# gpuopenanalytics/libgdf

Hardware: AMD Instinct MI355X
Metric: hash-join probe rows/s (higher is better)
Workload: dtype int64

## Files before the change

### libgdf_amd/csrc/join.hip

```cpp
#include "internal.h"
#include "launch.h"
#include "gdf/gdf_amd_ext.h"

#include <cmath>
#include <cstdio>

#include <algorithm>
#include <cstdlib>
#include <deque>
#include <memory>
#include <type_traits>
#include <vector>

namespace gdf_amd {

enum KeyMode : int { KM_RAW_INT = 0, KM_RAW_FLOAT, KM_PACKED, KM_HASHED };

struct KeyPlan {
  int mode;
  int verify;
  int narrow;
  uint64_t kmin;
  uint64_t kspan;
  uint64_t klimit;
// ... 1215 lines not shown
      tiles = (next - first + tile - 1) / tile;
    }
    uint32_t total;
    const uint32_t before = bk_block_scan<uint32_t>(tiles, lds_wave, &total);
    if (c < ncoarse) { coarse_off[c] = first; tile_prefix[c] = run + before; }
    run += total;
    block_sync();
  }
  if (threadIdx.x == 0) { coarse_off[ncoarse] = total_rows; tile_prefix[ncoarse] = run; }
  for (uint32_t f = threadIdx.x; f < nfine; f += JK_BK_THREADS) cursor[f] = begin[f];
}

struct Unit {
  uint32_t build_begin, build_count;
  uint32_t probe_begin, probe_count;
};

__global__ __launch_bounds__(256) void jk_make_units(uint32_t nfine, uint32_t cap2, const uint32_t *__restrict__ cursor,
                                                     const uint32_t *__restrict__ level1_flag,
                                                     const uint32_t *__restrict__ build_begin, const uint32_t *__restrict__ build_cnt,
                                                     int keep_probe, Unit *__restrict__ units, uint64_t *__restrict__ off,
                                                     unsigned long long *__restrict__ state, const uint32_t *__restrict__ fstart = nullptr,
                                                     const uint32_t *__restrict__ fcap = nullptr) {
  const uint32_t f = blockIdx.x * 256 + threadIdx.x;
  const uint32_t fc = f < nfine ? f : nfine - 1;
  const uint32_t cur = cursor[fc], bn = build_cnt[fc], bb = build_begin[fc];
  const uint32_t first = fstart ? fstart[fc] : fc * cap2;
  if (fcap) cap2 = fcap[fc];
  const uint32_t grown = f < nfine ? cur - first : 0u;
  const uint32_t all = grown < cap2 ? grown : cap2;
  const uint32_t pn = (all != 0 && (bn != 0 || keep_probe)) ? all : 0u;
  const uint32_t nun = (pn + JK_PROBE_CHUNK - 1) / JK_PROBE_CHUNK;
  const uint32_t incl_u = wave_scan_incl(nun);
  const unsigned long long incl_t = wave_scan_incl((unsigned long long)pn);
  const unsigned long long sum_all = wave_reduce_add((unsigned long long)all);
  unsigned long long base_u = 0, base_t = 0;
  if (lane_id() == WAVE - 1) {
    if (incl_u) { base_u = atomicAdd(&state[0], (unsigned long long)incl_u); base_t = atomicAdd(&state[1], incl_t); }
    if (sum_all) atomicAdd(&state[2], sum_all);
  }
  base_u = __shfl(base_u, WAVE - 1, WAVE);
  base_t = __shfl(base_t, WAVE - 1, WAVE);
  unsigned long long u = base_u + incl_u - nun, o = base_t + incl_t - pn;
  for (uint32_t at = 0; at < pn; at += JK_PROBE_CHUNK) {
    const uint32_t cnt = pn - at < JK_PROBE_CHUNK ? pn - at : JK_PROBE_CHUNK;
    units[u] = Unit{bb, bn, first + at, cnt};
    off[u] = o;
    ++u;
    o += cnt;
  }
  if (f == 0) state[3] = (unsigned long long)((cursor[nfine] ? 1u : 0u) | ((level1_flag && *level1_flag) ? 2u : 0u));
}

struct ProbeArgs {
  Tuples build, probe;
  const Unit *units;
  uint32_t nslots;
  uint32_t cap;
  int keep_unmatched_probe;
  int verify;
  uint8_t *build_matched;
  uint64_t *counts;
  int32_t *out_probe; int32_t *out_build;
  int unused;
  uint64_t kbias;
  int optimistic;
  unsigned long long *opt_state;
  uint32_t *unit_todo;
  uint32_t sample_n;
  const unsigned long long *nunits_dev;
  uint32_t *unit_pairs;
  int pay_mode;
  const void *pay_src[2];
  void *pay_out[2];
  int key_width;
  const void *key_src;
  void *key_out;
  int bpay_mode;
  const void *bpay_src[2];
  void *bpay_out[2];
  int p6_fb;
  uint32_t p6_world;
  uint64_t p6_kbias;
};
__device__ __forceinline__ void pay_gather(const ProbeArgs &a, unsigned long long pos, int32_t prow) {
  if (a.pay_mode == 1 || a.pay_mode == 4) {
    ((uint64_t *)a.pay_out[0])[pos] = ((const uint64_t *)a.pay_src[0])[prow];
    if (a.pay_mode == 4) ((uint64_t *)a.pay_out[1])[pos] = ((const uint64_t *)a.pay_src[1])[prow];
  } else if (a.pay_mode) {
    ((uint32_t *)a.pay_out[0])[pos] = ((const uint32_t *)a.pay_src[0])[prow];
    if (a.pay_mode == 3) ((uint32_t *)a.pay_out[1])[pos] = ((const uint32_t *)a.pay_src[1])[prow];
  }
  if (a.key_width == 8) ((uint64_t *)a.key_out)[pos] = ((const uint64_t *)a.key_src)[prow];
  else if (a.key_width == 4) ((uint32_t *)a.key_out)[pos] = ((const uint32_t *)a.key_src)[prow];
}
__device__ __forceinline__ void bpay_gather(const ProbeArgs &a, unsigned long long pos, int32_t brow) {
  if (a.bpay_mode == 1 || a.bpay_mode == 4) {
    ((uint64_t *)a.bpay_out[0])[pos] = ((const uint64_t *)a.bpay_src[0])[brow];
    if (a.bpay_mode == 4) ((uint64_t *)a.bpay_out[1])[pos] = ((const uint64_t *)a.bpay_src[1])[brow];
  } else if (a.bpay_mode) {
    ((uint32_t *)a.bpay_out[0])[pos] = ((const uint32_t *)a.bpay_src[0])[brow];
    if (a.bpay_mode == 3) ((uint32_t *)a.bpay_out[1])[pos] = ((const uint32_t *)a.bpay_src[1])[brow];
  }
}

struct ProbeLds {
  uint64_t *bw;
  uint32_t *T;
  int32_t *bi;
  unsigned long long *wave_cnt;
  unsigned long long *unit_cursor;
  unsigned int *cuckoo_failed;
  uint32_t *next;
};

template <bool NARROW>
__device__ __forceinline__ ProbeLds carve_probe_lds(unsigned char *raw, uint32_t cap, uint32_t H) {
  ProbeLds l;
  l.bw = (uint64_t *)raw;
  l.T = (uint32_t *)(raw + (size_t)cap * 8);
  unsigned char *after = raw + (size_t)cap * 8 + (size_t)H * 8;
  l.bi = (int32_t *)after;
  if (!NARROW) after += (size_t)cap * 4;
  l.wave_cnt = (unsigned long long *)after;
  l.unit_cursor = l.wave_cnt + JK_PROBE_THREADS / WAVE;
  l.cuckoo_failed = (unsigned int *)(l.unit_cursor + 1);
  l.next = (uint32_t *)(l.unit_cursor + 2);
  return l;
}
static size_t probe_lds_bytes(bool narrow, uint32_t cap, uint32_t H, bool chained = true) {
  return (size_t)cap * (narrow ? 8 : 12) + (size_t)H * 8 + sizeof(unsigned long long) * (JK_PROBE_THREADS / WAVE + 2) +
         (chained ? (size_t)cap * 4 : 0);
}

template <bool NARROW>
__device__ __forceinline__ int32_t build_row(const ProbeLds &l, uint32_t p) {
  return NARROW ? (int32_t)(uint32_t)l.bw[p] : l.bi[p];
}

template <bool WRITE, bool NARROW, bool P6 = false>
__global__ __launch_bounds__(JK_PROBE_THREADS) void jk_probe(ProbeArgs a, KeyTable probe_t, KeyTable build_t) {
  extern __shared__ __attribute__((aligned(16))) unsigned char lds_raw[];
  const uint32_t H = a.nslots, cap = a.cap;
  const ProbeLds l = carve_probe_lds<NARROW>(lds_raw, cap, H);
  uint32_t uid = a.unit_todo ? a.unit_todo[blockIdx.x] : blockIdx.x;
  if (a.sample_n) {
    const unsigned long long nunits = *a.nunits_dev;
    if (nunits == 0) return;
    uid = (uint32_t)(((unsigned long long)blockIdx.x * nunits) / a.sample_n);
  }
  const Unit u = a.units[uid];

  for (uint32_t i = threadIdx.x; i < u.build_count; i += JK_PROBE_THREADS) {
    uint64_t w = a.build.w[u.build_begin + i];
    if constexpr (P6 && NARROW) w = ((uint64_t)p6_remainder((uint32_t)(w >> 32), a.p6_kbias, a.p6_fb, a.p6_world) << 32) | (uint32_t)w;
    else if constexpr (P6) w = p10_key(w + a.p6_kbias, a.p6_fb);
    l.bw[i] = w;
    if (!NARROW) l.bi[i] = a.build.idx[u.build_begin + i];
  }
  for (uint32_t i = threadIdx.x; i < 2 * H; i += JK_PROBE_THREADS) l.T[i] = JK_NOPOS;
  __shared__ uint32_t dup_seen;
  if (threadIdx.x == 0) { *l.unit_cursor = WRITE ? a.counts[uid] : 0ull; *l.cuckoo_failed = 0; dup_seen = 0; }
  block_sync();

  for (uint32_t p0 = threadIdx.x; p0 < u.build_count; p0 += JK_PROBE_THREADS) {
    uint32_t cur = p0, table = 0;
// ... 140 lines not shown
          }
        }
      }
    }
#pragma unroll
    for (int b = 0; b < NB; ++b) {
      const bool active = act[b];
      uint32_t c = cnt[b];
      const bool pad = active && c == 0 && a.keep_unmatched_probe;
      if (pad) c = 1;
      if (!WRITE) {
        my_count += c;
      } else {
        unsigned long long pos;
        if (__all(c <= 1)) {
          const unsigned long long mm = __ballot(c == 1);
          unsigned long long wbase = 0;
          if (lane_id() == 0 && mm) wbase = atomicAdd(l.unit_cursor, (unsigned long long)__popcll(mm));
          pos = __shfl(wbase, 0, WAVE) + mask_rank(mm);
        } else {
          const uint32_t incl = wave_scan_incl(c);
          const uint32_t wave_total = __shfl(incl, WAVE - 1, WAVE);
          unsigned long long wbase = 0;
          if (lane_id() == 0) wbase = atomicAdd(l.unit_cursor, (unsigned long long)wave_total);
          pos = __shfl(wbase, 0, WAVE) + incl - c;
        }
        if (pos + c > unit_end) {
          if (c) a.opt_state[1] = 1;
        } else if (pad) {
          a.out_probe[pos] = prow[b];
          a.out_build[pos] = JK_EMPTY;
          pay_gather(a, pos, prow[b]);
        } else if (c >= 1 && (cuckoo || c == 1)) {
          a.out_probe[pos] = prow[b];
          a.out_build[pos] = build_row<NARROW>(l, hit_a[b]);
          pay_gather(a, pos, prow[b]);
          bpay_gather(a, pos, build_row<NARROW>(l, hit_a[b]));
          if (c == 2) {
            a.out_probe[pos + 1] = prow[b];
            a.out_build[pos + 1] = build_row<NARROW>(l, hit_b[b]);
            pay_gather(a, pos + 1, prow[b]);
            bpay_gather(a, pos + 1, build_row<NARROW>(l, hit_b[b]));
          }
        } else if (c > 1) {
          for (uint32_t p = hit_b[b]; p != JK_NOPOS; p = l.next[p]) {
            if (!a.verify || rows_equal(probe_t, prow[b], build_t, build_row<NARROW>(l, p))) {
              a.out_probe[pos] = prow[b];
              a.out_build[pos] = build_row<NARROW>(l, p);
              pay_gather(a, pos, prow[b]);
              bpay_gather(a, pos, build_row<NARROW>(l, p));
              ++pos;
            }
          }
        }
      }
    }
  }
  if (WRITE && a.optimistic) {
    block_sync();
    if (threadIdx.x == 0) {
      atomicAdd(&a.opt_state[0], *l.unit_cursor - unit_base);
      if (a.unit_pairs) a.unit_pairs[uid] = (uint32_t)(*l.unit_cursor - unit_base);
    }
  }
  if (!WRITE) {
    my_count = wave_reduce_add(my_count);
    if (lane_id() == 0) l.wave_cnt[threadIdx.x / WAVE] = my_count;
    block_sync();
    if (threadIdx.x == 0) {
      unsigned long long t = 0;
      for (int w = 0; w < JK_PROBE_THREADS / WAVE; ++w) t += l.wave_cnt[w];
      if (a.sample_n) { atomicAdd(&a.opt_state[0], t); atomicAdd(&a.opt_state[1], (unsigned long long)u.probe_count); }
      else a.counts[uid] = t;
    }
  }
}

template <bool POW2, bool KEEP, bool NARROW, int PMODE = 0, bool P6 = false>
__global__ __launch_bounds__(JK_PROBE_THREADS) void jk_probe_fast(ProbeArgs a) {
  extern __shared__ __attribute__((aligned(16))) unsigned char lds_raw[];
  const uint32_t H = a.nslots, cap = a.cap;
  const ProbeLds l = carve_probe_lds<NARROW>(lds_raw, cap, H);
  unsigned int *lcur = (unsigned int *)l.unit_cursor;
  const Unit u = a.units[blockIdx.x];
  for (uint32_t i = threadIdx.x; i < u.build_count; i += JK_PROBE_THREADS) {
    uint64_t w = a.build.w[u.build_begin + i];
    if constexpr (P6 && NARROW) w = ((uint64_t)p6_remainder((uint32_t)(w >> 32), a.p6_kbias, a.p6_fb, a.p6_world) << 32) | (uint32_t)w;
    else if constexpr (P6) w = p10_key(w + a.p6_kbias, a.p6_fb);
    l.bw[i] = w;
    if (!NARROW) l.bi[i] = a.build.idx[u.build_begin + i];
  }
  for (uint32_t i = threadIdx.x; i < 2 * H; i += JK_PROBE_THREADS) l.T[i] = JK_NOPOS;
  if (threadIdx.x == 0) { *lcur = 0; *l.cuckoo_failed = 0; }
  block_sync();
  const uint32_t kb_lo = (uint32_t)a.kbias, kb_hi = (uint32_t)(a.kbias >> 32);
  using Key = typename std::conditional<NARROW, uint32_t, uint64_t>::type;
  auto fold_of = [&](Key key) -> uint32_t {
    if constexpr (P6 && !NARROW) {
      uint32_t x = (uint32_t)(key >> 32);
      x ^= x << 13;
      x ^= x >> 7;
      return x ^ (uint32_t)key;
    } else if constexpr (P6) {
      uint32_t x = (uint32_t)key;
      x ^= x << 13;
      x ^= x >> 7;
      return x;
    } else if constexpr (NARROW) {
      const uint32_t lo = key + kb_lo;
      const uint32_t hi = kb_hi + (lo < key ? 1u : 0u);
      return lo ^ (hi * 0x9e3779b1u);
    } else {
      return key_fold(key + a.kbias);
    }
  };
  auto fold2_of = [&](Key key, uint32_t f1) -> uint32_t {
    if constexpr (NARROW) return f1;
    else if constexpr (P6) {
      uint32_t x = (uint32_t)(key >> 32);
      x ^= x << 13;
      x ^= x >> 7;
      return __builtin_rotateleft32(x, 16) + (uint32_t)key + ((uint32_t)key << 3);
    } else return key_fold2(key + a.kbias);
  };
  auto staged_key = [&](uint32_t p) -> Key {
    if constexpr (NARROW) return (uint32_t)(l.bw[p] >> 32);
    else return l.bw[p];
  };
  const int hshift = POW2 ? 32 - (__ffs((int)H) - 1) : 0;
  uint32_t seed = 0;
  for (int attempt = 0; attempt < 4; ++attempt) {
    for (uint32_t p0 = threadIdx.x; p0 < u.build_count; p0 += JK_PROBE_THREADS) {
      uint32_t cur = p0, table = 0;
      int moves = 0;
      for (; moves < JK_CUCKOO_MAX_MOVES; ++moves) {
        const Key ck = staged_key(cur);
        const uint32_t f = fold_of(ck) ^ seed, f2 = fold2_of(ck, fold_of(ck)) ^ seed;
        const uint32_t slot = table ? H + (POW2 ? (f2 * 0xc2b2ae35u) >> hshift : __umulhi(f2 * 0xc2b2ae35u, H))
                                    : (POW2 ? (f * 0x9e3779b1u) >> hshift : __umulhi(f * 0x9e3779b1u, H));
        const uint32_t old = atomicExch(&l.T[slot], cur);
        if (old == JK_NOPOS) break;
        cur = old;
        table ^= 1;
      }
      if (moves == JK_CUCKOO_MAX_MOVES) *l.cuckoo_failed = 1;
    }
    block_sync();
    if (!*l.cuckoo_failed || attempt == 3) break;
    block_sync();
    for (uint32_t i = threadIdx.x; i < 2 * H; i += JK_PROBE_THREADS) l.T[i] = JK_NOPOS;
    if (threadIdx.x == 0) *l.cuckoo_failed = 0;
    seed += 0x9e3779b9u;
    block_sync();
  }
  if (*l.cuckoo_failed) {
    if (threadIdx.x == 0) a.unit_todo[atomicAdd(&a.opt_state[2], 1ull)] = blockIdx.x;
    return;
  }
  const unsigned long long unit_base = a.counts[blockIdx.x];
  const uint32_t unit_cap = a.optimistic ? u.probe_count : 0xffffffffu;
  int32_t *__restrict__ op = a.out_probe + unit_base;
  int32_t *__restrict__ ob = a.out_build + unit_base;
  constexpr int NB = JK_PROBE_BATCH * 2;
  const uint32_t lead = u.probe_begin & 1u;
  const uint64_t *__restrict__ src = a.probe.w + (u.probe_begin - lead);
  const int32_t *__restrict__ src_row = NARROW ? nullptr : a.probe.idx + (u.probe_begin - lead);
  const uint64_t *__restrict__ src_pay = PMODE ? a.probe.pay + (size_t)(u.probe_begin - lead) * (PMODE == 4 ? 2 : 1) : nullptr;
  uint64_t *__restrict__ po8 = (PMODE == 1 || PMODE == 4) ? (uint64_t *)a.pay_out[0] + unit_base : nullptr;
  uint64_t *__restrict__ po8b = PMODE == 4 ? (uint64_t *)a.pay_out[1] + unit_base : nullptr;
  uint32_t *__restrict__ po4a = (PMODE == 2 || PMODE == 3) ? (uint32_t *)a.pay_out[0] + unit_base : nullptr;
  uint32_t *__restrict__ po4b = PMODE == 3 ? (uint32_t *)a.pay_out[1] + unit_base : nullptr;
  uint64_t *__restrict__ ko8 = (PMODE && a.key_width == 8) ? (uint64_t *)a.key_out + unit_base : nullptr;
  uint32_t *__restrict__ ko4 = (PMODE && a.key_width == 4) ? (uint32_t *)a.key_out + unit_base : nullptr;
  const uint32_t vtotal = lead + u.probe_count;
  const uint32_t last_pair = (vtotal - 1) & ~1u;
  for (uint32_t base = 0; base < vtotal; base += JK_PROBE_THREADS * NB) {
    Key key[NB];
    uint32_t prow[NB];
    uint64_t pay[PMODE ? NB : 1], pay2[PMODE == 4 ? NB : 1];
    bool act[NB];
#pragma unroll
    for (int b = 0; b < JK_PROBE_BATCH; ++b) {
      const uint32_t v = base + (b * JK_PROBE_THREADS + threadIdx.x) * 2;
      const uint32_t vc = v < last_pair ? v : last_pair;
      ulonglong2 ww{};
      if constexpr (P6) {
        uint32_t r0, row0, r1, row1;
        p6_load_pair(a.probe.w, (u.probe_begin - lead) + vc, r0, row0, r1, row1);
        if constexpr (NARROW) {
          key[2 * b] = r0; key[2 * b + 1] = r1;
        } else {
          const HiPair hh = *reinterpret_cast<const HiPair *>(a.probe.idx + (u.probe_begin - lead) + vc);
          key[2 * b] = ((uint64_t)r0 << 32) | hh.a; key[2 * b + 1] = ((uint64_t)r1 << 32) | hh.b;
        }
        prow[2 * b] = row0; prow[2 * b + 1] = row1;
      } else {
        ww = *reinterpret_cast<const ulonglong2 *>(src + vc);
      }
      if constexpr (PMODE == 4) {
        const ulonglong2 p0 = *reinterpret_cast<const ulonglong2 *>(src_pay + 2 * (size_t)vc);
        const ulonglong2 p1 = *reinterpret_cast<const ulonglong2 *>(src_pay + 2 * (size_t)vc + 2);
        pay[2 * b] = p0.x; pay2[2 * b] = p0.y; pay[2 * b + 1] = p1.x; pay2[2 * b + 1] = p1.y;
      } else if constexpr (PMODE != 0) {
        const ulonglong2 pp = *reinterpret_cast<const ulonglong2 *>(src_pay + vc);
        pay[2 * b] = pp.x; pay[2 * b + 1] = pp.y;
      }
      if constexpr (P6) {
      } else if constexpr (NARROW) {
        key[2 * b] = (uint32_t)(ww.x >> 32); prow[2 * b] = (uint32_t)ww.x;
        key[2 * b + 1] = (uint32_t)(ww.y >> 32); prow[2 * b + 1] = (uint32_t)ww.y;
      } else {
        const uint2 rr = *reinterpret_cast<const uint2 *>(src_row + vc);
        key[2 * b] = ww.x; prow[2 * b] = rr.x;
        key[2 * b + 1] = ww.y; prow[2 * b + 1] = rr.y;
      }
      act[2 * b] = v >= lead && v < vtotal;
      act[2 * b + 1] = v + 1 < vtotal;
    }
    uint32_t pa[NB], pb[NB];
#pragma unroll
    for (int b = 0; b < NB; ++b) {
      const uint32_t f = fold_of(key[b]) ^ seed, f2 = fold2_of(key[b], fold_of(key[b])) ^ seed;
      pa[b] = l.T[POW2 ? (f * 0x9e3779b1u) >> hshift : __umulhi(f * 0x9e3779b1u, H)];
      pb[b] = l.T[H + (POW2 ? (f2 * 0xc2b2ae35u) >> hshift : __umulhi(f2 * 0xc2b2ae35u, H))];
    }
    uint64_t wa[NB], wb[NB];
#pragma unroll
    for (int b = 0; b < NB; ++b) {
      wa[b] = l.bw[pa[b] == JK_NOPOS ? 0 : pa[b]];
      wb[b] = l.bw[pb[b] == JK_NOPOS ? 0 : pb[b]];
    }
    uint32_t hamask = 0, hbmask = 0, padmask = 0;
#pragma unroll
    for (int b = 0; b < NB; ++b) {
      const bool ha = act[b] && pa[b] != JK_NOPOS && (NARROW ? (uint32_t)(wa[b] >> 32) == (uint32_t)key[b] : wa[b] == (uint64_t)key[b]);
      const bool hb = act[b] && pb[b] != JK_NOPOS && (NARROW ? (uint32_t)(wb[b] >> 32) == (uint32_t)key[b] : wb[b] == (uint64_t)key[b]);
      hamask |= (uint32_t)ha << b;
      hbmask |= (uint32_t)hb << b;
      padmask |= (uint32_t)(KEEP && act[b] && !ha && !hb) << b;
    }
    int32_t hitrow[NARROW ? 1 : NB];
    if constexpr (!NARROW) {
#pragma unroll
      for (int b = 0; b < NB; ++b) {
        const bool ha = (hamask >> b) & 1u, hb = (hbmask >> b) & 1u;
        hitrow[b] = l.bi[ha ? pa[b] : (hb ? pb[b] : 0u)];
      }
    }
    auto emit = [&](int b, uint32_t pos, uint32_t c) {
      const bool ha = (hamask >> b) & 1u, pad = (padmask >> b) & 1u;
      if (pos + c > unit_cap) a.opt_state[1] = 1;
      else {
        int32_t first;
        if constexpr (NARROW) first = ha ? (int32_t)(uint32_t)wa[b] : (int32_t)(uint32_t)wb[b];
        else first = hitrow[b];
        op[pos] = (int32_t)prow[b];
        ob[pos] = pad ? JK_EMPTY : first;
        if (c == 2) {
          op[pos + 1] = (int32_t)prow[b];
          if constexpr (NARROW) ob[pos + 1] = (int32_t)(uint32_t)wb[b];
          else ob[pos + 1] = l.bi[pb[b]];
        }
        if constexpr (PMODE == 1 || PMODE == 4) { po8[pos] = pay[b]; if (c == 2) po8[pos + 1] = pay[b]; }
        if constexpr (PMODE == 4) { po8b[pos] = pay2[b]; if (c == 2) po8b[pos + 1] = pay2[b]; }
        if constexpr (PMODE == 2 || PMODE == 3) { po4a[pos] = (uint32_t)pay[b]; if (c == 2) po4a[pos + 1] = (uint32_t)pay[b]; }
        if constexpr (PMODE == 3) { po4b[pos] = (uint32_t)(pay[b] >> 32); if (c == 2) po4b[pos + 1] = (uint32_t)(pay[b] >> 32); }
        if constexpr (PMODE != 0 && NARROW) {
          if (ko8) { ko8[pos] = (uint64_t)key[b] + a.kbias; if (c == 2) ko8[pos + 1] = (uint64_t)key[b] + a.kbias; }
          if (ko4) { ko4[pos] = (uint32_t)key[b]; if (c == 2) ko4[pos + 1] = (uint32_t)key[b]; }
        }
      }
    };
    if (__all((hamask & hbmask) == 0)) {
      const uint32_t onemask = hamask | hbmask | padmask;
      unsigned long long mm[NB];
      uint32_t off[NB], tot = 0;
#pragma unroll
      for (int b = 0; b < NB; ++b) {
        mm[b] = __ballot((onemask >> b) & 1u);
        off[b] = tot;
        tot += (uint32_t)__popcll(mm[b]);
      }
      uint32_t wbase = 0;
      if (lane_id() == 0 && tot) wbase = atomicAdd(lcur, tot);
      wbase = (uint32_t)__builtin_amdgcn_readfirstlane((int)wbase);
#pragma unroll
      for (int b = 0; b < NB; ++b)
        if ((onemask >> b) & 1u) emit(b, wbase + off[b] + (uint32_t)mask_rank(mm[b]), 1u);
    } else {
#pragma unroll
      for (int b = 0; b < NB; ++b) {
        const uint32_t c = ((hamask >> b) & 1u) + ((hbmask >> b) & 1u) + ((padmask >> b) & 1u);
        uint32_t pos;
        if (__all(c <= 1)) {
          const unsigned long long mm = __ballot(c == 1);
          uint32_t wbase = 0;
          if (lane_id() == 0 && mm) wbase = atomicAdd(lcur, (unsigned int)__popcll(mm));
          pos = __shfl(wbase, 0, WAVE) + mask_rank(mm);
        } else {
          const uint32_t incl = wave_scan_incl(c);
          const uint32_t wave_total = __shfl(incl, WAVE - 1, WAVE);
          uint32_t wbase = 0;
          if (lane_id() == 0) wbase = atomicAdd(lcur, wave_total);
          pos = __shfl(wbase, 0, WAVE) + incl - c;
        }
        if (c) emit(b, pos, c);
      }
    }
  }
  if (a.optimistic) {
    block_sync();
    if (threadIdx.x == 0) {
      atomicAdd(&a.opt_state[0], (unsigned long long)*lcur);
      if (a.unit_pairs) a.unit_pairs[blockIdx.x] = *lcur;
    }
  }
}

template <bool POW2, bool KEEP, bool NARROW, bool P6 = false>
__global__ __launch_bounds__(JK_PROBE_THREADS) void jk_count_fast(ProbeArgs a) {
  extern __shared__ __attribute__((aligned(16))) unsigned char lds_raw[];
  const uint32_t H = a.nslots, cap = a.cap;
  const ProbeLds l = carve_probe_lds<NARROW>(lds_raw, cap, H);
  const Unit u = a.units[blockIdx.x];
  for (uint32_t i = threadIdx.x; i < u.build_count; i += JK_PROBE_THREADS) {
    uint64_t w = a.build.w[u.build_begin + i];
    if constexpr (P6 && NARROW) w = ((uint64_t)p6_remainder((uint32_t)(w >> 32), a.p6_kbias, a.p6_fb, a.p6_world) << 32) | (uint32_t)w;
    else if constexpr (P6) w = p10_key(w + a.p6_kbias, a.p6_fb);
    l.bw[i] = w;
    if (!NARROW) l.bi[i] = a.build.idx[u.build_begin + i];
  }
  for (uint32_t i = threadIdx.x; i < 2 * H; i += JK_PROBE_THREADS) l.T[i] = JK_NOPOS;
  if (threadIdx.x == 0) *l.cuckoo_failed = 0;
  block_sync();
  const uint32_t kb_lo = (uint32_t)a.kbias, kb_hi = (uint32_t)(a.kbias >> 32);
  using Key = typename std::conditional<NARROW, uint32_t, uint64_t>::type;
  auto fold_of = [&](Key key) -> uint32_t {
    if constexpr (P6 && !NARROW) {
      uint32_t x = (uint32_t)(key >> 32);
      x ^= x << 13;
      x ^= x >> 7;
      return x ^ (uint32_t)key;
    } else if constexpr (P6) {
      uint32_t x = (uint32_t)key;
      x ^= x << 13;
      x ^= x >> 7;
      return x;
    } else if constexpr (NARROW) {
      const uint32_t lo = key + kb_lo;
      const uint32_t hi = kb_hi + (lo < key ? 1u : 0u);
      return lo ^ (hi * 0x9e3779b1u);
    } else {
      return key_fold(key + a.kbias);
    }
  };
  auto fold2_of = [&](Key key, uint32_t f1) -> uint32_t {
    if constexpr (NARROW) return f1;
    else if constexpr (P6) {
      uint32_t x = (uint32_t)(key >> 32);
      x ^= x << 13;
      x ^= x >> 7;
      return __builtin_rotateleft32(x, 16) + (uint32_t)key + ((uint32_t)key << 3);
    } else return key_fold2(key + a.kbias);
  };
  auto staged_key = [&](uint32_t p) -> Key {
    if constexpr (NARROW) return (uint32_t)(l.bw[p] >> 32);
    else return l.bw[p];
  };
  const int hshift = POW2 ? 32 - (__ffs((int)H) - 1) : 0;
  uint32_t seed = 0;
  for (int attempt = 0; attempt < 4; ++attempt) {
    for (uint32_t p0 = threadIdx.x; p0 < u.build_count; p0 += JK_PROBE_THREADS) {
      uint32_t cur = p0, table = 0;
      int moves = 0;
      for (; moves < JK_CUCKOO_MAX_MOVES; ++moves) {
        const Key ck = staged_key(cur);
        const uint32_t f = fold_of(ck) ^ seed, f2 = fold2_of(ck, fold_of(ck)) ^ seed;
        const uint32_t slot = table ? H + (POW2 ? (f2 * 0xc2b2ae35u) >> hshift : __umulhi(f2 * 0xc2b2ae35u, H))
                                    : (POW2 ? (f * 0x9e3779b1u) >> hshift : __umulhi(f * 0x9e3779b1u, H));
        const uint32_t old = atomicExch(&l.T[slot], cur);
        if (old == JK_NOPOS) break;
        cur = old;
        table ^= 1;
      }
      if (moves == JK_CUCKOO_MAX_MOVES) *l.cuckoo_failed = 1;
    }
    block_sync();
    if (!*l.cuckoo_failed || attempt == 3) break;
    block_sync();
// ... 1225 lines not shown
    sb->pay[0].reset();
    if (flag) return GDF_SUCCESS;
    if (app) {
      app->rows += n;
      *ok = true;
      return GDF_SUCCESS;
    }
    sb->fine_begin.resize(nfine);
    sb->fine_cnt.resize(nfine);
    for (uint32_t f = 0; f < nfine; ++f) { sb->fine_begin[f] = f * cap2; sb->fine_cnt[f] = cur[f] - f * cap2; }
    sb->final_buf = 1;
  }
  uint64_t total = 0;
  for (uint32_t c : sb->fine_cnt) total += c;
  sb->joinable = (uint32_t)total;
  sb->speculative = true;
  *ok = true;
  return GDF_SUCCESS;
}

static gdf_error spec_append_finish(const PartGeom &g, SpecAppend *app, SideBufs *sb) {
  const uint32_t nfine = 1u << g.fb;
  std::vector<uint32_t> cur(nfine);
  HIP_TRY(read_back(cur.data(), app->cursor.p, sizeof(uint32_t) * nfine));
  sb->fine_off.clear();
  sb->fine_begin.resize(nfine);
  sb->fine_cnt.resize(nfine);
  uint64_t total = 0;
  for (uint32_t f = 0; f < nfine; ++f) {
    sb->fine_begin[f] = f * app->cap2;
    sb->fine_cnt[f] = cur[f] - f * app->cap2;
    total += sb->fine_cnt[f];
  }
  sb->final_buf = 1;
  sb->joinable = (uint32_t)total;
  sb->speculative = true;
  return GDF_SUCCESS;
}

static gdf_error run_probe(bool narrow, bool write, const char *name, size_t nunits, size_t lds, const ProbeArgs &a,
                           const KeyTable &probe_t, const KeyTable &build_t) {
  if (!nunits) return GDF_SUCCESS;
  GDF_TRY(with_bools([&](auto W, auto N, auto P6) {
    return launch_lds(name, jk_probe<W(), N(), P6()>, dim3((unsigned)nunits), dim3(JK_PROBE_THREADS), lds, a, probe_t, build_t);
  }, write, narrow, a.p6_fb != 0));
  HIP_CHECK_LAST();
  return GDF_SUCCESS;
}

static bool lean_table(uint32_t max_build, ProbeArgs *fa) {
  const bool pow2 = (double)max_build <= 0.42 * 2.0 * (double)fa->nslots;
  if (!pow2) fa->nslots = ((uint32_t)(max_build * 1.25) + 63) & ~63u;
  return pow2;
}

static gdf_error run_write_pass(bool narrow, bool plain, size_t nunits, size_t lds, ProbeArgs a, uint32_t max_build,
                                const KeyTable &probe_t, const KeyTable &build_t) {
  if (!nunits) return GDF_SUCCESS;
  if (!plain)
    return run_probe(narrow, true, "jk_probe_write", nunits, lds, a, probe_t, build_t);
  DevBuf todo;
  RMM_TRY(todo.alloc(sizeof(uint32_t) * nunits));
  a.unit_todo = todo.as<uint32_t>();
  ProbeArgs fa = a;
  const bool pow2 = lean_table(max_build, &fa);
  const size_t flds = probe_lds_bytes(narrow, a.cap, fa.nslots, false);
  const bool keep = a.keep_unmatched_probe != 0;
  auto lean = [&](auto N, auto M, auto P6) {
    return with_bools([&](auto P2, auto KP) {
      return launch_lds("jk_probe_write", jk_probe_fast<P2(), KP(), N(), M(), P6()>, dim3((unsigned)nunits), dim3(JK_PROBE_THREADS), flds, fa);
    }, pow2, keep);
  };
  constexpr std::true_type yes{};
  constexpr std::false_type no{};
  constexpr std::integral_constant<int, 0> none{};
  if (narrow && a.bpay_mode && !keep) {
    const bool bw2 = a.bpay_mode == 4;
    const size_t blds = probe_bp_lds_bytes(a.cap, fa.nslots, bw2);
    GDF_TRY(with_bools([&](auto P2, auto B2) {
      return with_int<0, 1, 2>(pay_words(a.pay_mode), [&](auto PP) {
        return launch_lds("jk_probe_write", jk_probe_bp<P2(), PP(), B2()>, dim3((unsigned)nunits), dim3(JK_BP_THREADS), blds, fa);
      });
    }, pow2, bw2));
  } else if (narrow && a.p6_fb) {
    GDF_TRY(lean(yes, none, yes));
  } else if (narrow && a.pay_mode) {
    GDF_TRY(with_int<1, 2, 3, 4>(a.pay_mode, [&](auto M) { return lean(yes, M, no); }));
  } else if (narrow) {
    GDF_TRY(lean(yes, none, no));
  } else {
    GDF_TRY(with_bools([&](auto P6) { return lean(no, none, P6); }, a.p6_fb != 0));
  }
  HIP_CHECK_LAST();
  unsigned long long left = 0;
  HIP_TRY(read_back(&left, a.opt_state + 2, sizeof(left)));
  if (left) GDF_TRY(run_probe(narrow, true, "jk_probe_write_general", (size_t)left, lds, a, probe_t, build_t));
  HIP_TRY(hipStreamSynchronize(stream0()));
  return GDF_SUCCESS;
}

static gdf_error run_multi_pass(bool write, size_t nunits, size_t lds, const ProbeArgs &a) {
  if (!nunits) return GDF_SUCCESS;
  GDF_TRY(with_bools([&](auto W, auto KP, auto SIX) {
    return launch_lds(write ? "jk_probe_write" : "jk_probe_count", jk_probe_multi<W(), KP(), SIX()>, dim3((unsigned)nunits), dim3(JK_PROBE_THREADS), lds, a);
  }, write, a.keep_unmatched_probe != 0, a.p6_fb != 0));
  HIP_CHECK_LAST();
  return GDF_SUCCESS;
}

static gdf_error run_count_pass(bool narrow, bool plain, size_t nunits, size_t lds, ProbeArgs a, uint32_t max_build,
                                const KeyTable &probe_t, const KeyTable &build_t) {
  if (!nunits) return GDF_SUCCESS;
  if (!plain || a.build_matched)
    return run_probe(narrow, false, "jk_probe_count", nunits, lds, a, probe_t, build_t);
  DevBuf todo;
  RMM_TRY(todo.alloc(sizeof(uint32_t) * nunits));
  a.unit_todo = todo.as<uint32_t>();
  ProbeArgs fa = a;
  const bool pow2 = lean_table(max_build, &fa);
  const size_t flds = probe_lds_bytes(narrow, a.cap, fa.nslots, false);
  GDF_TRY(with_bools([&](auto P2, auto KP, auto N, auto P6) {
    return launch_lds("jk_probe_count", jk_count_fast<P2(), KP(), N(), P6()>, dim3((unsigned)nunits), dim3(JK_PROBE_THREADS), flds, fa);
  }, pow2, a.keep_unmatched_probe != 0, narrow, a.p6_fb != 0));
  HIP_CHECK_LAST();
  unsigned long long left = 0;
  HIP_TRY(read_back(&left, a.opt_state + 2, sizeof(left)));
  if (left) GDF_TRY(run_probe(narrow, false, "jk_probe_count_general", (size_t)left, lds, a, probe_t, build_t));
  HIP_TRY(hipStreamSynchronize(stream0()));
  return GDF_SUCCESS;
}

static gdf_error refine_side(const PartGeom &g, bool narrow, double dup, SideBufs *sb, bool *ok) {
  *ok = false;
  const uint32_t nseg = 1u << g.fb, nsub = 1u << g.b3;
  const uint64_t nfine3 = (uint64_t)nseg << g.b3;
  const int64_t n = sb->joinable;
  if (n == 0) return GDF_SUCCESS;
  const int64_t TILE = (int64_t)JK_SC2_THREADS * (sb->pay[sb->final_buf].p ? JK_PAY_ITEMS : JK_SC_ITEMS);
  const double mean = (double)n / (double)nfine3;
  const uint32_t cap3 = (uint32_t)(((uint64_t)(mean + 8.0 * std::sqrt(mean * (1.0 + dup)) + 64.0) + 7) / 8 * 8);
  const uint64_t size3 = nfine3 * cap3 + TILE;
  if (size3 >= 0x7fffffffULL) return GDF_SUCCESS;
  std::vector<uint32_t> seg(2 * (size_t)nseg), tile_prefix((size_t)nseg + 1), cur((size_t)nfine3);
  tile_prefix[0] = 0;
  for (uint32_t c = 0; c < nseg; ++c) {
    seg[c] = sb->fine_begin[c];
    seg[nseg + c] = sb->fine_begin[c] + sb->fine_cnt[c];
    tile_prefix[c + 1] = tile_prefix[c] + (uint32_t)((sb->fine_cnt[c] + TILE - 1) / TILE);
  }
  for (uint64_t f = 0; f < nfine3; ++f) cur[f] = (uint32_t)(f * cap3);
  const uint32_t ntiles = tile_prefix[nseg];
  DevBuf d_seg, d_tiles, cursor, flag, nw, nidx, npay;
  const bool carries = sb->pay[sb->final_buf].p != nullptr;
  RMM_TRY(d_seg.alloc(sizeof(uint32_t) * 2 * nseg));
  RMM_TRY(d_tiles.alloc(sizeof(uint32_t) * ((size_t)nseg + 1)));
  RMM_TRY(cursor.alloc(sizeof(uint32_t) * nfine3));
  RMM_TRY(flag.alloc(sizeof(uint32_t)));
  RMM_TRY(nw.alloc(sizeof(uint64_t) * size3));
  if (!narrow) RMM_TRY(nidx.alloc(sizeof(int32_t) * size3));
  if (carries) RMM_TRY(npay.alloc(sizeof(uint64_t) * sb->pay_words * size3));
  HIP_TRY(hipMemcpyAsync(d_seg.p, seg.data(), sizeof(uint32_t) * 2 * nseg, hipMemcpyHostToDevice, stream0()));
  HIP_TRY(hipMemcpyAsync(d_tiles.p, tile_prefix.data(), sizeof(uint32_t) * ((size_t)nseg + 1), hipMemcpyHostToDevice, stream0()));
  HIP_TRY(hipMemcpyAsync(cursor.p, cur.data(), sizeof(uint32_t) * nfine3, hipMemcpyHostToDevice, stream0()));
  HIP_TRY(hipMemsetAsync(flag.p, 0, sizeof(uint32_t), stream0()));
  PartGeom g3 = g;
  g3.b1 = g.fb;
// ... 1881 lines not shown
```

Measured before the change: 109.9 billion.

## Add bitmap-rank probe kernel replacing cuckoo table for dense narrow keys

Adds a probe kernel that builds a per-unit LDS bitmap with prefix counts over key remainders, so each probe is a direct bit test plus popcount rank instead of a two-table cuckoo lookup. Units whose remainders collide fall back to the existing cuckoo kernel through a new unit list, and then to the general path. The aim is to remove cuckoo insertion cost and double-slot probing. The trade-offs are a large fixed LDS footprint, which lowers residency, and an extra readback and launch whenever any unit has duplicate remainders.

Measured after the change: 103.1 billion. -6.3%, worse.

```diff
diff --git a/libgdf_amd/csrc/join.hip b/libgdf_amd/csrc/join.hip
--- a/libgdf_amd/csrc/join.hip
+++ b/libgdf_amd/csrc/join.hip
@@ -1321,6 +1321,7 @@
   int p6_fb;
   uint32_t p6_world;
   uint64_t p6_kbias;
+  const uint32_t *unit_list;
 };
 __device__ __forceinline__ void pay_gather(const ProbeArgs &a, unsigned long long pos, int32_t prow) {
   if (a.pay_mode == 1 || a.pay_mode == 4) {
@@ -1627,7 +1628,8 @@
   const uint32_t H = a.nslots, cap = a.cap;
   const ProbeLds l = carve_probe_lds<NARROW>(lds_raw, cap, H);
   unsigned int *lcur = (unsigned int *)l.unit_cursor;
-  const Unit u = a.units[blockIdx.x];
+  const uint32_t uid = a.unit_list ? a.unit_list[blockIdx.x] : blockIdx.x;
+  const Unit u = a.units[uid];
   for (uint32_t i = threadIdx.x; i < u.build_count; i += JK_PROBE_THREADS) {
     uint64_t w = a.build.w[u.build_begin + i];
     if constexpr (P6 && NARROW) w = ((uint64_t)p6_remainder((uint32_t)(w >> 32), a.p6_kbias, a.p6_fb, a.p6_world) << 32) | (uint32_t)w;
@@ -1699,10 +1701,10 @@
     block_sync();
   }
   if (*l.cuckoo_failed) {
-    if (threadIdx.x == 0) a.unit_todo[atomicAdd(&a.opt_state[2], 1ull)] = blockIdx.x;
+    if (threadIdx.x == 0) a.unit_todo[atomicAdd(&a.opt_state[2], 1ull)] = uid;
     return;
   }
-  const unsigned long long unit_base = a.counts[blockIdx.x];
+  const unsigned long long unit_base = a.counts[uid];
   const uint32_t unit_cap = a.optimistic ? u.probe_count : 0xffffffffu;
   int32_t *__restrict__ op = a.out_probe + unit_base;
   int32_t *__restrict__ ob = a.out_build + unit_base;
@@ -1850,6 +1852,189 @@
           pos = __shfl(wbase, 0, WAVE) + incl - c;
         }
         if (c) emit(b, pos, c);
+      }
+    }
+  }
+  if (a.optimistic) {
+    block_sync();
+    if (threadIdx.x == 0) {
+      atomicAdd(&a.opt_state[0], (unsigned long long)*lcur);
+      if (a.unit_pairs) a.unit_pairs[uid] = *lcur;
+    }
+  }
+}
+
+constexpr int JK_RANK_BITS = 32 - JK_MAX_FB;
+constexpr uint32_t JK_RANK_WORDS = 1u << (JK_RANK_BITS - 5);
+constexpr int JK_RANK_STAGE = (JK_MAX_BUILD + JK_PROBE_THREADS - 1) / JK_PROBE_THREADS;
+constexpr bool JK_RANK_PACKED = false;
+constexpr int JK_RANK_BATCH = 4;
+constexpr int JK_RANK_RESIDENT = 2;
+static_assert(JK_RANK_WORDS % JK_PROBE_THREADS == 0 && JK_RANK_WORDS / JK_PROBE_THREADS == 8, "a thread owns 8 consecutive bitmap words");
+static_assert(JK_MAX_BUILD <= 0xffff, "the prefix of a bitmap word is a u16");
+static size_t rank_lds_bytes(uint32_t cap, bool packed) {
+  return (size_t)JK_RANK_WORDS * (packed ? 8 : 6) + (size_t)cap * 4 + sizeof(uint32_t) * (JK_PROBE_THREADS / WAVE + 4);
+}
+static size_t rank_launch_lds(uint32_t cap, bool packed) {
+  return std::max(rank_lds_bytes(cap, packed), (size_t)160 * 1024 / (JK_RANK_RESIDENT + 1) + 64);
+}
+template <bool KEEP, bool PACKED>
+__global__ __launch_bounds__(JK_PROBE_THREADS) void jk_probe_rank(ProbeArgs a) {
+  extern __shared__ __attribute__((aligned(16))) unsigned char lds_raw[];
+  constexpr int WORDS_PER_THREAD = JK_RANK_WORDS / JK_PROBE_THREADS;
+  uint2 *ent = (uint2 *)lds_raw;
+  uint32_t *bits = (uint32_t *)lds_raw;
+  uint16_t *pre = (uint16_t *)(lds_raw + (size_t)JK_RANK_WORDS * 4);
+  int32_t *brow = (int32_t *)(lds_raw + (size_t)JK_RANK_WORDS * (PACKED ? 8 : 6));
+  uint32_t *wave_sum = (uint32_t *)(brow + a.cap);
+  unsigned int *lcur = wave_sum + JK_PROBE_THREADS / WAVE;
+  unsigned int *repeated = lcur + 1;
+  const Unit u = a.units[blockIdx.x];
+  const uint32_t room = a.cap < (uint32_t)(JK_RANK_STAGE * JK_PROBE_THREADS) ? a.cap : (uint32_t)(JK_RANK_STAGE * JK_PROBE_THREADS);
+  const uint32_t bn = u.build_count < room ? u.build_count : room;
+  uint64_t bw[JK_RANK_STAGE];
+  if (bn) {
+#pragma unroll
+    for (int k = 0; k < JK_RANK_STAGE; ++k) {
+      const uint32_t i = k * JK_PROBE_THREADS + threadIdx.x;
+      bw[k] = a.build.w[u.build_begin + (i < bn ? i : bn - 1)];
+    }
+  } else {
+#pragma unroll
+    for (int k = 0; k < JK_RANK_STAGE; ++k) bw[k] = 0;
+  }
+  const uint32_t w0 = threadIdx.x * WORDS_PER_THREAD;
+  if constexpr (PACKED) {
+#pragma unroll
+    for (int j = 0; j < WORDS_PER_THREAD; j += 2) *reinterpret_cast<uint4 *>(&ent[w0 + j]) = uint4{0, 0, 0, 0};
+  } else {
+    *reinterpret_cast<uint4 *>(&bits[w0]) = uint4{0, 0, 0, 0};
+    *reinterpret_cast<uint4 *>(&bits[w0 + 4]) = uint4{0, 0, 0, 0};
+  }
+  if (threadIdx.x == 0) { *lcur = 0; *repeated = 0; }
+  block_sync();
+  uint32_t rem[JK_RANK_STAGE];
+  bool twice = false;
+#pragma unroll
+  for (int k = 0; k < JK_RANK_STAGE; ++k) {
+    rem[k] = p6_remainder((uint32_t)(bw[k] >> 32), a.p6_kbias, a.p6_fb, a.p6_world);
+    if (k * JK_PROBE_THREADS + threadIdx.x < bn) {
+      const uint32_t bit = 1u << (rem[k] & 31u);
+      const uint32_t old = PACKED ? atomicOr(&ent[rem[k] >> 5].x, bit) : atomicOr(&bits[rem[k] >> 5], bit);
+      twice |= (old & bit) != 0;
+    }
+  }
+  if (twice) *repeated = 1;
+  block_sync();
+  if (*repeated) {
+    if (threadIdx.x == 0) a.unit_todo[atomicAdd(&a.opt_state[3], 1ull)] = blockIdx.x;
+    return;
+  }
+  {
+    uint32_t wd[WORDS_PER_THREAD], mine = 0;
+#pragma unroll
+    for (int j = 0; j < WORDS_PER_THREAD; ++j) {
+      wd[j] = PACKED ? ent[w0 + j].x : bits[w0 + j];
+      mine += (uint32_t)__popc(wd[j]);
+    }
+    const uint32_t incl = wave_scan_incl(mine);
+    if (lane_id() == WAVE - 1) wave_sum[threadIdx.x / WAVE] = incl;
+    block_sync();
+    uint32_t run = incl - mine;
+#pragma unroll
+    for (int w = 0; w < JK_PROBE_THREADS / WAVE; ++w)
+      if (w < (int)(threadIdx.x / WAVE)) run += wave_sum[w];
+    if constexpr (PACKED) {
+#pragma unroll
+      for (int j = 0; j < WORDS_PER_THREAD; ++j) {
+        ent[w0 + j].y = run;
+        run += (uint32_t)__popc(wd[j]);
+      }
+    } else {
+      uint32_t packed[WORDS_PER_THREAD / 2];
+#pragma unroll
+      for (int j = 0; j < WORDS_PER_THREAD; j += 2) {
+        const uint32_t lo = run;
+        run += (uint32_t)__popc(wd[j]);
+        packed[j / 2] = lo | (run << 16);
+        run += (uint32_t)__popc(wd[j + 1]);
+      }
+      *reinterpret_cast<uint4 *>(&pre[w0]) = uint4{packed[0], packed[1], packed[2], packed[3]};
+    }
+  }
+  block_sync();
+  auto lookup = [&](uint32_t r, uint32_t &word, uint32_t &before) {
+    if constexpr (PACKED) {
+      const uint2 e = ent[r >> 5];
+      word = e.x;
+      before = e.y;
+    } else {
+      word = bits[r >> 5];
+      before = pre[r >> 5];
+    }
+  };
+  auto rank_of = [](uint32_t r, uint32_t word, uint32_t before) -> uint32_t {
+    return before + (uint32_t)__popc(word & ~(0xffffffffu << (r & 31u)));
+  };
+#pragma unroll
+  for (int k = 0; k < JK_RANK_STAGE; ++k) {
+    uint32_t word, before;
+    lookup(rem[k], word, before);
+    if (k * JK_PROBE_THREADS + threadIdx.x < bn) brow[rank_of(rem[k], word, before)] = (int32_t)(uint32_t)bw[k];
+  }
+  block_sync();
+  const unsigned long long unit_base = a.counts[blockIdx.x];
+  const uint32_t unit_cap = a.optimistic ? u.probe_count : 0xffffffffu;
+  int32_t *__restrict__ op = a.out_probe + unit_base;
+  int32_t *__restrict__ ob = a.out_build + unit_base;
+  constexpr int NB = JK_RANK_BATCH * 2;
+  const uint32_t lead = u.probe_begin & 1u;
+  const uint32_t vtotal = lead + u.probe_count;
+  const uint32_t last_pair = (vtotal - 1) & ~1u;
+  for (uint32_t base = 0; base < vtotal; base += JK_PROBE_THREADS * NB) {
+    uint32_t key[NB], prow[NB];
+    bool act[NB];
+#pragma unroll
+    for (int b = 0; b < JK_RANK_BATCH; ++b) {
+      const uint32_t v = base + (b * JK_PROBE_THREADS + threadIdx.x) * 2;
+      const uint32_t vc = v < last_pair ? v : last_pair;
+      p6_load_pair(a.probe.w, (u.probe_begin - lead) + vc, key[2 * b], prow[2 * b], key[2 * b + 1], prow[2 * b + 1]);
+      act[2 * b] = v >= lead && v < vtotal;
+      act[2 * b + 1] = v + 1 < vtotal;
+    }
+    uint32_t word[NB], before[NB];
+#pragma unroll
+    for (int b = 0; b < NB; ++b) lookup(key[b], word[b], before[b]);
+    uint32_t hitmask = 0, padmask = 0;
+    int32_t hitrow[NB];
+#pragma unroll
+    for (int b = 0; b < NB; ++b) {
+      const bool hit = act[b] && ((word[b] >> (key[b] & 31u)) & 1u);
+      hitmask |= (uint32_t)hit << b;
+      padmask |= (uint32_t)(KEEP && act[b] && !hit) << b;
+      hitrow[b] = brow[hit ? rank_of(key[b], word[b], before[b]) : 0u];
+    }
+    const uint32_t onemask = hitmask | padmask;
+    unsigned long long mm[NB];
+    uint32_t off[NB], tot = 0;
+#pragma unroll
+    for (int b = 0; b < NB; ++b) {
+      mm[b] = __ballot((onemask >> b) & 1u);
+      off[b] = tot;
+      tot += (uint32_t)__popcll(mm[b]);
+    }
+    uint32_t wbase = 0;
+    if (lane_id() == 0 && tot) wbase = atomicAdd(lcur, tot);
+    wbase = (uint32_t)__builtin_amdgcn_readfirstlane((int)wbase);
+#pragma unroll
+    for (int b = 0; b < NB; ++b) {
+      if ((onemask >> b) & 1u) {
+        const uint32_t pos = wbase + off[b] + (uint32_t)mask_rank(mm[b]);
+        if (pos + 1 > unit_cap) a.opt_state[1] = 1;
+        else {
+          op[pos] = (int32_t)prow[b];
+          ob[pos] = ((padmask >> b) & 1u) ? JK_EMPTY : hitrow[b];
+        }
       }
     }
   }
@@ -3241,6 +3426,34 @@
         return launch_lds("jk_probe_write", jk_probe_bp<P2(), PP(), B2()>, dim3((unsigned)nunits), dim3(JK_BP_THREADS), blds, fa);
       });
     }, pow2, bw2));
+  } else if (narrow && a.p6_fb == JK_MAX_FB && a.cap <= (uint32_t)(JK_RANK_STAGE * JK_PROBE_THREADS) && !lab::path_on("GDF_JK_NO_RANK")) {
+    DevBuf rtodo;
+    RMM_TRY(rtodo.alloc(sizeof(uint32_t) * nunits));
+    ProbeArgs ra = a;
+    ra.unit_todo = rtodo.as<uint32_t>();
+    const size_t rlds = rank_launch_lds(a.cap, JK_RANK_PACKED);
+    GDF_TRY(with_bools([&](auto KP) {
+      return launch_lds("jk_probe_write", jk_probe_rank<KP(), JK_RANK_PACKED>, dim3((unsigned)nunits), dim3(JK_PROBE_THREADS), rlds, ra);
+    }, keep));
+    HIP_CHECK_LAST();
+    unsigned long long st[2] = {0, 0};
+    HIP_TRY(read_back(st, a.opt_state + 2, sizeof(st)));
+    const size_t repeated = (size_t)st[1];
+    unsigned long long left = 0;
+    if (repeated) {
+      fa.unit_list = rtodo.as<uint32_t>();
+      GDF_TRY(with_bools([&](auto P2, auto KP) {
+        return launch_lds("jk_probe_write_cuckoo", jk_probe_fast<P2(), KP(), true, 0, true>, dim3((unsigned)repeated), dim3(JK_PROBE_THREADS), flds, fa);
+      }, pow2, keep));
+      HIP_CHECK_LAST();
+      HIP_TRY(read_back(&left, a.opt_state + 2, sizeof(left)));
+      if (left) GDF_TRY(run_probe(narrow, true, "jk_probe_write_general", (size_t)left, lds, a, probe_t, build_t));
+    }
+    lab::note("jk.rank_units", (long long)(nunits - repeated));
+    lab::note("jk.rank_cuckoo_units", (long long)(repeated - (size_t)left));
+    lab::note("jk.rank_general_units", (long long)left);
+    HIP_TRY(hipStreamSynchronize(stream0()));
+    return GDF_SUCCESS;
   } else if (narrow && a.p6_fb) {
     GDF_TRY(lean(yes, none, yes));
   } else if (narrow && a.pay_mode) {
```
